# hammershock/3dgs-avatar-release

Hardware: AMD Instinct MI355X
Metric: render fps (fwd+bwd) @200k Gaussians 1024x1024 SH3 (higher is better)
Workload: dtype f32; 1 GPU; config3: 200k Gaussians, 1024x1024, SH deg 3, forward+backward; shs+scales+rotations inputs, L1 loss (L1 fused into the rasterizer: l1_target); tile_rect=1, l1=fused, long_lists=0, gaussians=200000, width=1024, height=1024, sh_degree=3, frames_per_rank=1857, total_frames=1857, ranks=1, backend=none, parallelism=frames sharded x1

## Files before the change

### 3dgs-avatar-release_amd/csrc/binning.hip

```cpp
#include "common.h"

__global__ __launch_bounds__(256) void first_pair_kernel(const uint32_t* __restrict__ tiles,
                                                         const uint32_t* __restrict__ wave_tiles, float* __restrict__ rec,
                                                         int P, unsigned long long* __restrict__ count,
                                                         unsigned long long* host_count) {
    __shared__ unsigned long long wb[4];
    const int tid = threadIdx.x, lane = tid & 63, wid = tid >> 6;
    const int w0 = 4 * (int)blockIdx.x;
    unsigned long long before = 0;
    for (int w = tid; w < w0; w += 256) before += wave_tiles[w];
#pragma unroll
    for (int d = 32; d >= 1; d >>= 1) before += __shfl_xor(before, d, 64);
    if (lane == 0) wb[wid] = before;
    const int i = blockIdx.x * 256 + tid;
    const uint32_t v = i < P ? tiles[i] : 0u;
    uint32_t x = v;
#pragma unroll
    for (int d = 1; d < 64; d <<= 1) {
        const uint32_t y = __shfl_up(x, d, 64);
        if (lane >= d) x += y;
    }
    __syncthreads();
    const unsigned long long block_base = (wb[0] + wb[1]) + (wb[2] + wb[3]);
    uint32_t woff = 0;
// ... 395 lines not shown
                                                          const uint32_t* __restrict__ keys, int mode, int ntiles,
                                                          uint32_t* __restrict__ order, const PairCount pc,
                                                          const FillJob fill, const LongLists ll) {
    if (blockIdx.x > 0) {
        if (fill.clean && *fill.clean == MARKS_CLEAN) return;
        const uint4 ones = make_uint4(0xFFFFFFFFu, 0xFFFFFFFFu, 0xFFFFFFFFu, 0xFFFFFFFFu);
        for (size_t k = (size_t)(blockIdx.x - 1) * 1024 + threadIdx.x; k < fill.quads; k += (size_t)(gridDim.x - 1) * 1024)
            if (fill.stream) store_stream(&fill.ptr[k], ones); else fill.ptr[k] = ones;
        return;
    }
    __shared__ uint32_t hist[1024];
    __shared__ uint32_t wmax[16];
    __shared__ uint32_t wsum[16];
    if (mode < 0) return;
    tile_order_body<HELD>(ranges, keys, mode, ntiles, order, pc, ll, hist, wmax, wsum);
}

#define BM_LD 33
#ifndef TW_STOP_AFTER
#define TW_STOP_AFTER 99
#endif
template <bool CW>
__global__ __launch_bounds__(TBK_THREADS) void tile_write_kernel(const uint4* __restrict__ ranklist,
                                                                 const uint32_t* __restrict__ seg_start, int P, int gx,
                                                                 int gy, int nbx, int nblocks, int nseg, int ntiles,
                                                                 const uint32_t* __restrict__ seg_cnt,
                                                                 const uint32_t* __restrict__ tile_tot,
                                                                 uint2* __restrict__ ranges, uint32_t* __restrict__ order,
                                                                 uint32_t* __restrict__ point_list, const PairCount pc,
                                                                 const LongLists ll) {
// ... 197 lines not shown

int launch_tile_order(const uint32_t* ranges, const uint32_t* keys, int mode, int ntiles, uint32_t* order, PairCount pc,
                      FillJob fill, LongLists ll, int debug, hipStream_t s) {
    const size_t pieces = (fill.quads + 1023) / 1024;
    const int side = fill.ptr ? (int)(pieces < 255 ? pieces : 255) : 0;
    if (ntiles <= 32 * 1024)
        hipLaunchKernelGGL(tile_order_kernel<true>, dim3(1 + side), dim3(1024), 0, s, reinterpret_cast<const uint2*>(ranges),
                           keys, mode, ntiles, order, pc, fill, ll);
    else
        hipLaunchKernelGGL(tile_order_kernel<false>, dim3(1 + side), dim3(1024), 0, s, reinterpret_cast<const uint2*>(ranges),
                           keys, mode, ntiles, order, pc, fill, ll);
    GS_LAUNCH_CHECK("tile_order", debug, s);
    return GS_OK;
}

int launch_tile_lists(const uint4* ranklist, const uint32_t* chunk_pairs, uint32_t* seg_start, int P, int gx, int gy, TileCounts tc, uint32_t* ranges,
                      uint32_t* order, uint32_t* point_list, PairCount pc, LongLists ll, bool totals_zeroed, int debug,
                      hipStream_t s) {
    uint32_t* seg_cnt = tc.seg_cnt;
    const BinGrid G = bin_grid(gx, gy);
    const int nseg = bin_segments(G, P);
    const int ntiles = gx * gy;
    if (!totals_zeroed) {
        const int zrc = gs_zero_async(tc.tile_tot, tc.zero_bytes, "tile_totals.zero", s);
        if (zrc != GS_OK) return zrc;
    }
    {
        int band_rows = TC_CELLS / (gx + 1) - 1;
        if (band_rows < 1) return GS_E_TOO_LARGE;
        if (band_rows > gy) band_rows = gy;
// ... 21 lines not shown
```

### 3dgs-avatar-release_amd/csrc/capi.hip

```cpp
#include "common.h"
#include <string.h>
#include <stdlib.h>
#include <atomic>
#include <chrono>
#include <mutex>
#include <vector>

static thread_local int g_last_hip = 0;
static thread_local const char* g_last_stage = "";
void gs_set_error(int hip_err, const char* stage) {
    g_last_hip = hip_err;
    g_last_stage = stage;
}

struct TuneSwitch {
    const char* name;
    int key, def;
    const char* env;
    bool (*ok)(int);
};
static const TuneSwitch k_tune[GS_TUNE_COUNT] = {
    {"xcd_map", GS_TUNE_XCD_MAP, 1, nullptr, nullptr},
    {"depth_sort", GS_TUNE_DEPTH_SORT, 1, nullptr, nullptr},
    {"nt_stores", GS_TUNE_NT_STORES, 1, nullptr, nullptr},
    {"bwd_chunks", GS_TUNE_BWD_CHUNKS, 1, nullptr, nullptr},
    {"fwd4", GS_TUNE_FWD4, 1, "GSPLAT_FWD4", nullptr},
    {"small_tiles", GS_TUNE_SMALL_TILES, BWD_CHUNK_MAX_TILES, nullptr, nullptr},
    {"shared_qlist", GS_TUNE_SHARED_QLIST, 1, nullptr, nullptr},
    {"ones_fast", GS_TUNE_ONES_FAST, 1, nullptr, nullptr},
    {"bwd_order", GS_TUNE_BWD_ORDER, 1, nullptr, nullptr},
    {"fwd_marks", GS_TUNE_FWD_MARKS, 1, nullptr, nullptr},
    {"fwdc_ch", GS_TUNE_FWDC_CH, (int)FWDC_CH_MIN, "GSPLAT_FWDC_CH", [](int v) { return v >= 64 && (v & (v - 1)) == 0; }},
    {"fwdc_div", GS_TUNE_FWDC_DIV, (int)FWD4_TOTAL_DIV, "GSPLAT_FWDC_DIV", [](int v) { return v >= 1; }},
};
struct TuneState {
    std::atomic<int> v[GS_TUNE_COUNT];
    TuneState() {
        for (const TuneSwitch& t : k_tune) {
            int value = t.def;
            if (const char* e = t.env ? getenv(t.env) : nullptr) {
                const int x = atoi(e);
                if (!t.ok || t.ok(x)) value = x;
            }
            v[t.key].store(value);
        }
    }
};
static TuneState& tune_state() {
// ... 289 lines not shown
        StageScope sc_("ranges_order", s);
        rc = launch_tile_order(im.ranges, nullptr, 0, im.ntiles, im.order, pc, FillJob{nullptr, 0},
                               LongLists{0, nullptr, im.cw_hdr, nullptr}, a->debug, s);
        if (rc != GS_OK) return rc;
    }
    QuadLists ql = quad_lists(im, b, a->long_lists);
    if (chunked) quad_lists_chunked(ql, im, im);
    if (cap > 0) {
        ql.marks = (gs_tune_get(GS_TUNE_FWD_MARKS) && !a->forward_only) ? b.marks : nullptr;
        ql.mark_quads = (size_t)cap;
        ql.marks_flag = b.marks_flag;
    }
    ql.l1_target = a->l1_target;
    ql.l1_part = im.l1_part;
    ql.l1_loss = a->l1_loss;
    { StageScope sc_("render_fwd", s);
    rc = launch_render_forward(g.rec, a->P > 0 ? b.point_list : nullptr, im.ranges, im.order, a->bg, a->W, a->H, out_color,
                               im.final_T, im.n_contrib, ql, s); }
    if (rc != GS_OK) return rc;
    return sync_if_debug(a, "render_forward", s);
}

int gs_forward_render(const GsFwdArgs* a, void* geom, size_t geom_bytes, void* binning, size_t binning_bytes,
                      void* img, size_t img_bytes, int64_t D, float* out_color, void* stream) {
    GS_CAPTURE_OK_IF(stream, a && !a->debug && a->frame_stats == nullptr);
    return forward_phase2(a, geom, geom_bytes, binning, binning_bytes, img, img_bytes, D, out_color, stream, false);
}

int gs_forward(const GsFwdArgs* a, void* geom, size_t geom_bytes, void* binning, size_t binning_bytes, int64_t capacity,
               void* img, size_t img_bytes, int32_t* radii, int64_t* count_host_pinned, float* out_color,
// ... 122 lines not shown
    if (a->P > 0 && scratch_bytes < scratch_total_bytes(D, a->P, im.ntiles)) return GS_E_WORKSPACE;
    if (a->P == 0) return GS_OK;
    hipStream_t s = (hipStream_t)stream;
    float* const sums = (float*)((char*)scratch + scratch_rows_bytes(D));
    if (D > 0) {
        const QuadLists ql = quad_lists(im, b, a->long_lists);
        SecondImage si{nullptr, nullptr, nullptr, nullptr, nullptr};
        if (second) {
            const ImgViewRO im2 = img_state(second->img, a->W, a->H, second->long_lists);
            if (second->img_bytes < im2.total || im2.bwd_chunks != im.bwd_chunks) return GS_E_BAD_ARG;
            si = SecondImage{second->colors, second->out_color, second->dL_dpix, ql.chunks > 1 ? im2.ckpt : nullptr, im2.all_ones};
        }
        uint32_t* const q8 = reinterpret_cast<uint32_t*>(b.marks);
        uint32_t* const own_order = (uint32_t*)((char*)sums + scratch_sums_bytes(a->P));
        const bool order_here = gs_tune_get(GS_TUNE_BWD_ORDER) != 0;
        { StageScope sc_("tile_order", s);
        rc = launch_tile_order(im.ranges, ql.qcount, order_here ? 1 : -1, im.ntiles, own_order, PairCount{nullptr, 0},
                               FillJob{b.marks, (size_t)D, gs_tune_get(GS_TUNE_NT_STORES) & 1, b.marks_flag},
                               LongLists{0, nullptr}, a->debug, s); }
        if (rc != GS_OK) return rc;
        { StageScope sc_("render_bwd", s);
        rc = launch_render_backward(g.rec, im.ranges, order_here ? own_order : im.order, a->W, a->H, ql, out_color, dL_dpix,
                                    dL_dopacity_img, im.final_T, a->bg, (float*)scratch, q8, second ? &si : nullptr,
                                    L1Grad{a->l1_target, a->l1_grad}, s); }
        if (rc != GS_OK) return rc;
        rc = sync_if_debug(a, "render_backward", s);
        if (rc != GS_OK) return rc;
    }
    StageScope sc_("gaussian_bwd", s);
    return launch_gaussian_backward(*a, radii, g.rec, g.tiles, g.clamped, reinterpret_cast<const uint32_t*>(b.marks),
                                    (const float*)scratch, sums, b.marks_flag, *gr, s);
}

int gs_backward(const GsFwdArgs* a, const int32_t* radii, const void* geom, size_t geom_bytes, void* binning,
                size_t binning_bytes, const void* img, size_t img_bytes, int64_t D, const float* out_color,
                const float* dL_dpix, void* scratch, size_t scratch_bytes, const GsGrads* gr, void* stream) {
    return backward_impl(a, radii, geom, geom_bytes, binning, binning_bytes, img, img_bytes, D, out_color, dL_dpix, nullptr,
// ... 838 lines not shown
    *n_out = n;
    return GS_OK;
}

int gs_tuning(const char* name, int value) {
    if (!name) return GS_E_BAD_ARG;
    for (const TuneSwitch& t : k_tune) {
        if (strcmp(name, t.name) != 0) continue;
        if (t.ok && !t.ok(value)) return GS_E_BAD_ARG;
        tune_state().v[t.key].store(value);
        return GS_OK;
    }
    return GS_E_BAD_ARG;
}

const char* gs_status_string(int code) {
    switch (code) {
        case GS_OK: return "ok";
        case GS_E_BAD_ARG: return "bad argument (null required pointer, non-positive size, unsupported SH degree / more than 16 SH coefficients, or rotations not 16-byte aligned)";
        case GS_E_EXCLUSIVE: return "provide exactly one of shs/colors_precomp and exactly one of (scales, rotations)/cov3D_precomp";
        case GS_E_TOO_LARGE: return "num_rendered or tile grid exceeds the supported index space";
        case GS_E_HIP: return "HIP error";
        case GS_E_WORKSPACE: return "state/workspace buffer smaller than gs_*_bytes requires";
        case GS_E_CAPTURE: return "the stream is being captured into a graph and this call is not capture-safe with these arguments (include/gsplat_mi355.h, \"Stream capture\"); nothing was enqueued";
        default: return "unknown status";
    }
}
int gs_last_hip_error(void) { return g_last_hip; }
const char* gs_last_stage(void) { return g_last_stage; }
const char* gs_build_info(void) { return "gsplat_mi355 gfx950 wave64 tile16 rec48"; }
// ... 3 lines not shown
```

### 3dgs-avatar-release_amd/csrc/common.h

```cpp
#pragma once
#include <hip/hip_runtime.h>
#include <stdint.h>
#include <stddef.h>
#include <type_traits>
#include "../../include/gsplat_mi355.h"

#define TILE 16
#define WAVE 64
#define REC_F 12
#define GS_MAX_PAIRS 0x3FFFFFFFll

static inline size_t align_up(size_t x, size_t a) { return (x + a - 1) / a * a; }

#define SORT_ITEMS 4096
#define SORT_SMALL_N (1 << 20)
#define SORT_TOTALS_REPL 16
static inline size_t sort_table_words(size_t n) {
    const size_t items = n <= (size_t)SORT_SMALL_N ? 1024 : SORT_ITEMS;
    return (size_t)256 * ((n + items - 1) / items + 4 * SORT_TOTALS_REPL);
}
#define SCAN_ITEMS 2048

#ifndef DS_ITEMS
#define DS_ITEMS 2048
// ... 78 lines not shown
    G.nby = (gy + TB_H - 1) / TB_H;
    G.nblocks = G.nbx * G.nby;
#ifndef TB_TARGET_WGS
#define TB_TARGET_WGS 512
#endif
    int s = (TB_TARGET_WGS + G.nblocks - 1) / G.nblocks;
    G.nseg_max = s < 1 ? 1 : (s > TB_MAX_SEG ? TB_MAX_SEG : s);
    return G;
}
static inline int bin_segments(const BinGrid& G, int P) {
    int s = (P + 1023) / 1024;
    if (s < 1) s = 1;
    return s < G.nseg_max ? s : G.nseg_max;
}

enum { GS_TUNE_XCD_MAP = 0, GS_TUNE_DEPTH_SORT = 1, GS_TUNE_NT_STORES = 2, GS_TUNE_BWD_CHUNKS = 3, GS_TUNE_FWD4 = 4, GS_TUNE_SMALL_TILES = 5, GS_TUNE_SHARED_QLIST = 6, GS_TUNE_ONES_FAST = 7, GS_TUNE_BWD_ORDER = 8, GS_TUNE_FWD_MARKS = 9, GS_TUNE_FWDC_CH = 10, GS_TUNE_FWDC_DIV = 11, GS_TUNE_COUNT = 12 };
int gs_tune_get(int key);

#define BWD_CH 128
#define BWD_KMAX 16
#define BWD_CHUNK_MAX_TILES 2048
#define FWD4_MAX_TILES 2048
#define FWD4_MIN_LIST 512u
#ifndef FWD4_TOTAL_DIV
#define FWD4_TOTAL_DIV 320ull
#endif

#define FWDC_CH_MIN 256u
#define FWDC_SPARSE_PAIRS 524288ull
#define FWDC_MAX_UNITS 4096
#define FWDC_MAX_TILES (FWDC_MAX_UNITS / 2)
#define FWDC_Q_WORDS (8 * FWDC_MAX_UNITS * 4)
#define FWDC_Q_BYTES ((size_t)FWDC_Q_WORDS * 4 + 64)
#ifdef FWDC_PROF
#define FWDC_SLOTS 9
#else
#define FWDC_SLOTS 8
#endif
#define FWDC_DEAD 0x80000000u
#define FWDC_SPIN_MAX (1 << 16)
struct ImgLayout {
    size_t ranges, n_contrib, final_T, ncon_c, tile_nmax, order, seg_cnt, tile_tot, all_ones, cw_flag, cw_done, cw_q, tile_zero_bytes, l1_part, ckpt, ck_start, cw_hdr, cw_units, cw_items, cw_rec, total;
    int gx, gy, bwd_chunks;
};
static inline bool few_long_lists_mode(int ntiles, int long_lists) {
    return ntiles <= gs_tune_get(GS_TUNE_SMALL_TILES) || long_lists != 0;
}
static inline ImgLayout img_layout(int W, int H, int long_lists = 0) {
    ImgLayout L;
    size_t o = 0;
    auto take = [&](size_t bytes) { size_t at = o; o = align_up(o + bytes, 256); return at; };
    L.gx = (W + TILE - 1) / TILE;
    L.gy = (H + TILE - 1) / TILE;
    const size_t nt = (size_t)L.gx * L.gy;
    L.ranges = take(nt * 8);
    L.n_contrib = take((size_t)W * H * 4);
    L.final_T = take((size_t)W * H * 4);
// ... 12 lines not shown
        L.cw_done = take(nt * 16);
        L.cw_q = take(FWDC_Q_BYTES);
        L.tile_zero_bytes = L.cw_q + FWDC_Q_BYTES - L.tile_tot;
    }
    L.l1_part = take(nt * 16);
    L.bwd_chunks = fl ? BWD_KMAX : 1;
    L.ckpt = take(nt * 4 * (size_t)(L.bwd_chunks - 1) * 64 * 16);
    L.ck_start = take(nt * 4 * (size_t)L.bwd_chunks * 4);
    L.cw_hdr = L.cw_units = L.cw_items = L.cw_rec = 0;
    if (cw) {
        L.cw_hdr = take(64);
        L.cw_units = take((size_t)FWDC_MAX_UNITS * 8);
        L.cw_items = take((size_t)FWDC_Q_WORDS * 4);
        L.cw_rec = take((size_t)FWDC_MAX_UNITS * 4 * FWDC_SLOTS * 64 * 4);
    }
    L.total = o;
    return L;
}

template <bool RO>
struct StateCarve {
    typename std::conditional<RO, const char, char>::type* base;
    StateCarve(typename std::conditional<RO, const void, void>::type* state) : base(static_cast<decltype(base)>(state)) {}
    template <class T>
    void operator()(T*& field, size_t offset, bool present = true) const {
        field = (base && present) ? reinterpret_cast<T*>(base + offset) : nullptr;
    }
};
template <bool RO>
struct GeomViewT {
// ... 17 lines not shown
    size_t total;
};
template <bool RO>
struct ImgViewT {
    template <class T> using ptr = typename std::conditional<RO, const T, T>::type*;
    ptr<uint32_t> ranges, n_contrib;
    ptr<float> final_T;
    ptr<uint32_t> ncon_c, qcount , order, seg_cnt, tile_tot, all_ones;
    ptr<uint32_t> cw_flag, cw_done, cw_q, cw_xcc_mask ;
    ptr<float> l1_part;
    ptr<float4> ckpt;
    ptr<uint32_t> ck_start, cw_hdr;
    ptr<uint2> cw_units;
    ptr<uint32_t> cw_items;
    ptr<float> cw_rec;
    size_t tile_zero_bytes;
    int cw_clear_words;
    size_t total;
    int gx, gy, ntiles, bwd_chunks;
};
typedef GeomViewT<false> GeomView;
typedef GeomViewT<true> GeomViewRO;
typedef BinViewT<false> BinView;
typedef BinViewT<true> BinViewRO;
typedef ImgViewT<false> ImgView;
typedef ImgViewT<true> ImgViewRO;

template <class Void >
static inline GeomViewT<std::is_const<Void>::value> geom_state(Void* base, int P) {
    constexpr bool RO = std::is_const<Void>::value;
// ... 22 lines not shown
}
template <class Void >
static inline ImgViewT<std::is_const<Void>::value> img_state(Void* base, int W, int H, int long_lists) {
    constexpr bool RO = std::is_const<Void>::value;
    const ImgLayout L = img_layout(W, H, long_lists);
    const StateCarve<RO> at{base};
    const bool cw = L.cw_rec != 0;
    ImgViewT<RO> v;
    at(v.ranges, L.ranges); at(v.n_contrib, L.n_contrib); at(v.final_T, L.final_T); at(v.ncon_c, L.ncon_c);
    at(v.qcount, L.tile_nmax); at(v.order, L.order); at(v.seg_cnt, L.seg_cnt); at(v.tile_tot, L.tile_tot);
    at(v.all_ones, L.all_ones);
    at(v.cw_flag, L.cw_flag, cw); at(v.cw_done, L.cw_done, cw); at(v.cw_q, L.cw_q, cw);
    at(v.cw_xcc_mask, L.cw_q + (size_t)FWDC_Q_WORDS * 4, cw);
    at(v.l1_part, L.l1_part); at(v.ckpt, L.ckpt); at(v.ck_start, L.ck_start);
    at(v.cw_hdr, L.cw_hdr, cw); at(v.cw_units, L.cw_units, cw); at(v.cw_items, L.cw_items, cw); at(v.cw_rec, L.cw_rec, cw);
    v.tile_zero_bytes = L.tile_zero_bytes;
    v.cw_clear_words = cw ? (int)((L.cw_q + FWDC_Q_BYTES - L.cw_flag) / 4) : 0;
    v.total = L.total; v.gx = L.gx; v.gy = L.gy; v.ntiles = L.gx * L.gy; v.bwd_chunks = L.bwd_chunks;
    return v;
}
static inline unsigned long long* not_ones_word(const GeomViewRO& first) {
    return const_cast<unsigned long long*>(first.count) + COUNT_NOT_ONES;
}

static inline int radix_passes(int bits) { return (bits + 7) / 8; }

void gs_set_error(int hip_err, const char* stage);
#define GS_LAUNCH_CHECK(stage, dbg, stream)                                            \
    do {                                                                               \
        hipError_t e__ = hipGetLastError();                                            \
// ... 307 lines not shown
int launch_knn_points(int Nq, const float* queries, int Nr, const float* ref, int K, float* out_d, long long* out_i,
                      void* ws, size_t ws_bytes, hipStream_t s);

int launch_build_cov(int N, const float* scales, float mod, const float* rot, int is_matrix, float* cov6, hipStream_t s);
int launch_build_cov_bwd(int N, const float* scales, float mod, const float* rot, int is_matrix, const float* dL_dcov6,
                         float* dL_dscales, float* dL_drot, hipStream_t s);
int launch_sh2rgb(int N, int deg, int M, const float* shs, const float* xyz, const float* campos, const float* R_fwd,
                  const float* noise_host, float* colors, uint8_t* clamped, hipStream_t s);
int launch_sh2rgb_bwd(int N, int deg, int M, const float* shs, const float* xyz, const float* campos, const float* R_fwd,
                      const float* noise_host, const uint8_t* clamped, const float* dL_dcolors, float* dL_dshs, float* dL_dxyz,
                      hipStream_t s);

size_t l1_ws_bytes(int64_t n);
int launch_l1_loss(const float* x, const float* y, int64_t n, float* loss, float* grad, float* partial, hipStream_t s);
int launch_loss_final(const float* partial, int nparts, float inv_n, float* loss, hipStream_t s);
int launch_bce_loss(const float* x, const float* y, int64_t n, float* loss, float* grad, float* partial, hipStream_t s);
size_t ssim_ws_bytes(int C, int H, int W);
int launch_ssim_forward(int C, int H, int W, const float* img1, const float* img2, float* ssim_out, float* dm_dmu1,
                        float* dm_ds1, float* dm_ds12, float* partial, hipStream_t s);
int launch_ssim_backward(int C, int H, int W, const float* img1, const float* img2, const float* dm_dmu1,
                         const float* dm_ds1, const float* dm_ds12, const float* dL_dssim, float* dL_dimg1,
                         hipStream_t s);

#define MARKS_CLEAN 0x600DF111u
struct FillJob { uint4* ptr; size_t quads; int stream = 0; const uint32_t* clean = nullptr;  };

typedef uint32_t gs_u32x4 __attribute__((ext_vector_type(4)));
__device__ __forceinline__ void store_stream(uint4* p, uint4 v) {
    gs_u32x4 x = {v.x, v.y, v.z, v.w};
    __builtin_nontemporal_store(x, reinterpret_cast<gs_u32x4*>(p));
// ... 17 lines not shown
    const float* src_cw_rec = nullptr;
    const float* src_final_T = nullptr;
    const uint32_t* src_qcount = nullptr;
    const uint32_t* src_n_contrib = nullptr;
    const unsigned long long* not_ones = nullptr;
    float4* ckpt = nullptr;
    uint32_t* ck_start = nullptr;
    int chunks = 1;
    uint4* marks = nullptr;
    size_t mark_quads = 0;
    uint32_t* marks_flag = nullptr;
    uint32_t* all_ones = nullptr;
    const float* l1_target = nullptr;
    float* l1_part = nullptr;
    float* l1_loss = nullptr;
};
int launch_render_forward(const float* rec, const uint32_t* point_list, const uint32_t* ranges, const uint32_t* order,
                          const float* bg, int W, int H, float* out_color, float* final_T, uint32_t* n_contrib,
                          const QuadLists& ql, hipStream_t s);
struct SecondImage {
    const float* colors;
    const float* out_color;
    const float* dL_dpix;
    const float4* ckpt;
    const uint32_t* all_ones;
};
struct L1Grad { const float* target; const float* grad; };
int launch_render_backward(const float* rec, const uint32_t* ranges, const uint32_t* order, int W, int H,
                           const QuadLists& ql, const float* out_color, const float* dL_dpix, const float* dL_dopa,
                           const float* final_T, const float* bg, float* qrows, uint32_t* q8, const SecondImage* second,
// ... 20 lines not shown
```

### 3dgs-avatar-release_amd/csrc/loss.hip

```cpp
#include "common.h"
#include <math.h>

#define L1_THREADS 256
#define L1_MAX_BLOCKS 1024

__device__ __forceinline__ float sgn_over_n(float d, float inv_n) { return d > 0.f ? inv_n : (d < 0.f ? -inv_n : 0.f); }

__global__ __launch_bounds__(L1_THREADS) void l1_partial_kernel(const float* __restrict__ x, const float* __restrict__ y,
                                                                int64_t n, float inv_n, float* __restrict__ grad,
                                                                float* __restrict__ partial) {
    __shared__ float ws[L1_THREADS / 64];
    const int tid = threadIdx.x, lane = tid & 63, wid = tid >> 6;
    float acc = 0.f;
    const int64_t n4 = n >> 2;
    const float4* x4 = reinterpret_cast<const float4*>(x);
    const float4* y4 = reinterpret_cast<const float4*>(y);
    float4* g4 = reinterpret_cast<float4*>(grad);
    const int64_t stride = (int64_t)gridDim.x * L1_THREADS;
    for (int64_t i = (int64_t)blockIdx.x * L1_THREADS + tid; i < n4; i += stride) {
        const float4 a = x4[i], b = y4[i];
        const float d0 = a.x - b.x, d1 = a.y - b.y, d2 = a.z - b.z, d3 = a.w - b.w;
        acc += (fabsf(d0) + fabsf(d1)) + (fabsf(d2) + fabsf(d3));
        g4[i] = make_float4(sgn_over_n(d0, inv_n), sgn_over_n(d1, inv_n), sgn_over_n(d2, inv_n), sgn_over_n(d3, inv_n));
    }
// ... 50 lines not shown

int launch_bce_loss(const float* x, const float* y, int64_t n, float* loss, float* grad, float* partial, hipStream_t s) {
    const int blocks = l1_blocks(n);
    const float inv_n = 1.0f / (float)n;
    StageScope st("bce_loss", s);
    hipLaunchKernelGGL(bce_partial_kernel, dim3(blocks), dim3(L1_THREADS), 0, s, x, y, n, inv_n, grad, partial);
    GS_LAUNCH_CHECK("bce_loss.partial", 0, s);
    hipLaunchKernelGGL(l1_final_kernel, dim3(1), dim3(L1_THREADS), 0, s, partial, blocks, inv_n, loss);
    GS_LAUNCH_CHECK("bce_loss.final", 0, s);
    return GS_OK;
}

__global__ __launch_bounds__(1024) void loss_final_wide_kernel(const float* __restrict__ partial, int nparts, float inv_n,
                                                               float* __restrict__ loss) {
    __shared__ float ws[16];
    const int tid = threadIdx.x, lane = tid & 63, wid = tid >> 6;
    float acc = 0.f;
    for (int i0 = tid; i0 < nparts; i0 += 8 * 1024) {
        float v[8];
#pragma unroll
        for (int u = 0; u < 8; u++) v[u] = (i0 + u * 1024 < nparts) ? partial[i0 + u * 1024] : 0.f;
#pragma unroll
        for (int u = 0; u < 8; u++) acc += v[u];
    }
    acc = wave_sum(acc);
    if (lane == 0) ws[wid] = acc;
    __syncthreads();
    if (tid == 0) {
        float t = 0.f;
        for (int w = 0; w < 16; w++) t += ws[w];
        loss[0] = t * inv_n;
    }
}

int launch_loss_final(const float* partial, int nparts, float inv_n, float* loss, hipStream_t s) {
    hipLaunchKernelGGL(loss_final_wide_kernel, dim3(1), dim3(1024), 0, s, partial, nparts, inv_n, loss);
    GS_LAUNCH_CHECK("loss_final", 0, s);
    return GS_OK;
}

int launch_l1_loss(const float* x, const float* y, int64_t n, float* loss, float* grad, float* partial, hipStream_t s) {
    const int blocks = l1_blocks(n);
    const float inv_n = 1.0f / (float)n;
    StageScope st("l1_loss", s);
    hipLaunchKernelGGL(l1_partial_kernel, dim3(blocks), dim3(L1_THREADS), 0, s, x, y, n, inv_n, grad, partial);
    GS_LAUNCH_CHECK("l1_loss.partial", 0, s);
    hipLaunchKernelGGL(l1_final_kernel, dim3(1), dim3(L1_THREADS), 0, s, partial, blocks, inv_n, loss);
// ... 260 lines not shown
```

### 3dgs-avatar-release_amd/csrc/render_fwd.hip

```cpp
#include "common.h"
#include "blend.h"
#include <type_traits>

struct FwdArgs {
    const float4* __restrict__ rec;
    const uint32_t* __restrict__ point_list;
    const uint2* __restrict__ ranges;
    const uint32_t* __restrict__ order;
    const float* __restrict__ bg;
    int W, H, gx, ntiles, xmap;
    float* __restrict__ out_color;
    float* __restrict__ final_T;
    uint32_t* __restrict__ n_contrib;
    uint32_t* __restrict__ qlist;
    uint32_t* __restrict__ ncon_c;
    uint32_t* __restrict__ qcount;
    float4* __restrict__ ckpt;
    uint32_t* __restrict__ ck_start;
    int chunks;
    const uint32_t* __restrict__ src_qcount;
    const uint32_t* __restrict__ src_n_contrib;
    const unsigned long long* __restrict__ not_ones;
    uint4* __restrict__ marks;
    size_t mark_quads;
// ... 875 lines not shown
    const dim3 grid(render_grid_blocks(gx * gy, xmap) + A.cw_blocks);
    const bool fq = ql.src_qcount != nullptr;
    if (ql.four_waves) {
        if (fq) hipLaunchKernelGGL(render_fwd_small_kernel<true>, grid, dim3(FWD4_BATCH), 0, s, A);
        else hipLaunchKernelGGL(render_fwd_small_kernel<false>, grid, dim3(FWD4_BATCH), 0, s, A);
    } else {
        if (A.cw_blocks) {
            if (fq) hipLaunchKernelGGL(render_fwd_cw_kernel<true>, grid, dim3(64), 0, s, A);
            else hipLaunchKernelGGL(render_fwd_cw_kernel<false>, grid, dim3(64), 0, s, A);
        } else {
            if (fq) hipLaunchKernelGGL(render_fwd_kernel<true>, grid, dim3(64), 0, s, A);
            else hipLaunchKernelGGL(render_fwd_kernel<false>, grid, dim3(64), 0, s, A);
        }
    }
    GS_LAUNCH_CHECK("render_forward", 0, s);
    if (ql.l1_target)
        return launch_loss_final(ql.l1_part, gx * gy * 4, 1.0f / (3.0f * (float)W * (float)H), ql.l1_loss, s);
    return GS_OK;
}

__global__ __launch_bounds__(256) void opacity_image_kernel(const float* __restrict__ final_T, const float* __restrict__ bg,
                                                            int n, float* __restrict__ out) {
    const int i = blockIdx.x * blockDim.x + threadIdx.x;
    if (i >= n) return;
    const float Tf = final_T[i];
    out[i] = (1.0f - Tf) + Tf * bg[0];
}

int launch_opacity_image(const float* final_T, const float* bg, int W, int H, float* out, hipStream_t s) {
    const int n = W * H;
    hipLaunchKernelGGL(opacity_image_kernel, dim3((n + 255) / 256), dim3(256), 0, s, final_T, bg, n, out);
    GS_LAUNCH_CHECK("opacity_image", 0, s);
// ... 3 lines not shown
```

### 3dgs-avatar-release_amd/diff_gaussian_rasterization/__init__.py

```python
import ctypes
import os
import threading
import weakref
from typing import NamedTuple

import torch
import torch.nn as nn

from gsplat_mi355 import _lib

__all__ = ["GaussianRasterizationSettings", "GaussianRasterizer", "rasterize_gaussians"]


class GaussianRasterizationSettings(NamedTuple):
    image_height: int
    image_width: int
    tanfovx: float
    tanfovy: float
    bg: torch.Tensor
    scale_modifier: float
    viewmatrix: torch.Tensor
    projmatrix: torch.Tensor
    sh_degree: int
    campos: torch.Tensor
# ... 255 lines not shown
                                                cov3Ds_precomp, raster_settings, with_opacity, dep, l1_target)
        args = (means3D, means2D, sh, colors_precomp, opacities, scales, rotations, cov3Ds_precomp)
        try:
            return _RasterizeGaussians._forward(ctx, means3D, means2D, sh, colors_precomp, opacities, scales, rotations,
                                                cov3Ds_precomp, raster_settings, with_opacity, dep, l1_target)
        except Exception:
            _dump_snapshot("snapshot_fw.dump", raster_settings, args)
            print("\nAn error occured in forward. Please forward snapshot_fw.dump for debugging.")
            raise

    @staticmethod
    def _forward(ctx, means3D, means2D, sh, colors_precomp, opacities, scales, rotations, cov3Ds_precomp,
                 raster_settings, with_opacity=False, dep=None, l1_target=None):
        ctx.with_opacity = bool(with_opacity)
        ctx.l1_target = None
        l1 = None
        ctx.defer_to = None
        means2D_in = means2D
        ctx.set_materialize_grads(False)
        L = _lib.load()
        means3D = _f32c(means3D, "means3D")
        if means3D is None:
            raise RuntimeError("diff_gaussian_rasterization: means3D is empty")
        sh = _f32c(sh, "shs")
        colors_precomp = _f32c(colors_precomp, "colors_precomp")
        opacities = _f32c(opacities, "opacities")
        scales = _f32c(scales, "scales")
        rotations = _f32c(rotations, "rotations")
        if rotations is not None:
            rotations = _lib.contiguous_aligned(rotations)
# ... 5 lines not shown
        with _lib.on_device(dev):
            a = _make_args(raster_settings, means3D, sh, colors_precomp, opacities, scales, rotations, cov3Ds_precomp,
                           keep)
            stream_h = _lib.stream_handle(dev)
            sptr = ctypes.c_void_p(stream_h)
            capturing = _stream_capturing()
            if capturing:
                a.frame_stats = None
            if l1_target is not None:
                ctx.l1_target = l1_target
                l1 = torch.empty((), dtype=torch.float32, device=dev)
                a.l1_target, a.l1_loss = l1_target.data_ptr(), l1.data_ptr()
            inference = isinstance(ctx, _InferenceCtx)
            if inference:
                a.forward_only = 1
            share = _SHARE and not inference and any(ctx.needs_input_grad)
            gkey = (_geom_cache.key(raster_settings, means3D, opacities, scales, rotations, cov3Ds_precomp, stream_h,
                                    capturing)
                    if share else None)
            hit = _geom_cache.take(dev, gkey) if (share and l1_target is None) else None
            if not share or l1_target is not None:
                _geom_cache.offer.pop(dev.index, None)
            ctx.geom_entry = None
            if hit is not None:
                a.long_lists = int(hit.long_lists)
            geom_bytes = _size("gs_geom_bytes", P)
            ik = ("img", W, H, int(a.long_lists))
            img_bytes = _sizes.get(ik)
            if img_bytes is None:
                img_bytes = _sizes[ik] = _lib.nbytes(L.gs_image_bytes_for, ctypes.byref(a))
# ... 142 lines not shown
            grad_out_color = torch.zeros(3, H, W, dtype=torch.float32, device=dev)
        g = _f32c(grad_out_color, "grad_out_color") if grad_out_color is not None else None
        g_l1 = _f32c(grad_l1, "grad_l1") if use_l1 else None
        g_op = _f32c(grad_out_opacity, "grad_out_opacity") if (ctx.with_opacity and grad_out_opacity is not None) else None
        with _lib.on_device(dev):
            a, _keep = ctx.fwd_args
            if (a.means3D != means3D.data_ptr() or a.opacities != opacities.data_ptr()
                    or (has_sh and a.shs != sh.data_ptr()) or (has_sr and a.scales != scales.data_ptr())):
                _keep = []
                a = _make_args(settings, means3D, sh if has_sh else None, colors_precomp if has_col else None, opacities,
                               scales if has_sr else None, rotations if has_sr else None,
                               cov3Ds_precomp if has_cov else None, _keep, long_lists=ctx.long_lists)
            a.l1_target = ctx.l1_target.data_ptr() if use_l1 else None
            a.l1_loss = None
            a.l1_grad = g_l1.data_ptr() if use_l1 else None
            gp = g.data_ptr() if g is not None else None
            sptr = _lib.stream_ptr(dev)
            scratch_bytes = _size("gs_backward_scratch_bytes", D, P, W, H)
            scratch = torch.empty(scratch_bytes, dtype=torch.uint8, device=dev)
            M = int(sh.shape[1]) if has_sh else 0
            f = dict(dtype=torch.float32, device=dev)
            d_means3D = torch.empty(P, 3, **f)
            d_means2D = torch.empty(P, 3, **f)
            d_colors = torch.empty(P, 3, **f)
            d_opacity = torch.empty(P, 1, **f)
            d_cov3D = torch.empty(P, 6, **f)
            d_sh = torch.empty(P, M, 3, **f) if has_sh else None
            d_scales = torch.empty(P, 3, **f) if has_sr else None
            d_rot = torch.empty(P, 4, **f) if has_sr else None
            gr = _lib.GsGrads(_lib.ptr(d_means3D), _lib.ptr(d_means2D), _lib.ptr(d_sh), _lib.ptr(d_colors),
# ... 62 lines not shown
```

### 3dgs-avatar-release_amd/gsplat_mi355/_lib.py

```python
import ctypes
import os
import threading
from ctypes import POINTER, c_char_p, c_double, c_float, c_int, c_int32, c_int64, c_size_t, c_uint8, c_void_p

_HERE = os.path.dirname(os.path.abspath(__file__))
LIB_PATH = os.environ.get("GSPLAT_LIB_PATH") or os.path.join(os.path.dirname(_HERE), "lib", "libgsplat_mi355.so")


class GsFwdArgs(ctypes.Structure):
    _fields_ = [
        ("P", c_int32), ("sh_degree", c_int32), ("M", c_int32), ("W", c_int32), ("H", c_int32),
        ("bg", c_void_p), ("means3D", c_void_p), ("shs", c_void_p), ("colors_precomp", c_void_p),
        ("opacities", c_void_p), ("scales", c_void_p), ("rotations", c_void_p), ("cov3D_precomp", c_void_p),
        ("viewmatrix", c_void_p), ("projmatrix", c_void_p), ("campos", c_void_p),
        ("scale_modifier", c_float), ("tanfovx", c_float), ("tanfovy", c_float),
        ("prefiltered", c_int32), ("debug", c_int32), ("tile_rect", c_int32), ("long_lists", c_int32),
        ("frame_stats", c_void_p), ("l1_target", c_void_p), ("l1_loss", c_void_p), ("l1_grad", c_void_p),
        ("forward_only", c_int32),
    ]


class GsSecondImage(ctypes.Structure):
    _fields_ = [("colors", c_void_p), ("out_color", c_void_p), ("dL_dpix", c_void_p), ("img", c_void_p),
                ("img_bytes", c_size_t), ("long_lists", c_int32)]


class GsGrads(ctypes.Structure):
    _fields_ = [(n, c_void_p) for n in ("dL_dmeans3D", "dL_dmeans2D", "dL_dsh", "dL_dcolors", "dL_dopacity",
                                        "dL_dscales", "dL_drotations", "dL_dcov3D")]


EXPORTS = ["gs_geom_bytes", "gs_image_bytes", "gs_binning_bytes", "gs_backward_scratch_bytes",
           "gs_forward_preprocess", "gs_forward_render", "gs_forward", "gs_forward_shared", "gs_backward", "gs_mark_visible", "knn_workspace_bytes",
           "knn_dist2", "gs_geom_field", "gs_binning_field", "gs_image_field", "gs_status_string",
           "gs_last_hip_error", "gs_last_stage", "gs_build_info", "gs_profile_enable", "gs_profile_filter", "gs_profile_collect",
           "gs_l1_loss_workspace_bytes", "gs_l1_loss", "gs_bce_loss", "gs_ssim_workspace_bytes", "gs_ssim_forward", "gs_ssim_backward",
           "gs_build_covariance", "gs_build_covariance_backward", "gs_sh2rgb", "gs_sh2rgb_backward", "knn_points", "gs_densify_stats", "gs_adam_step",
           "gs_opacity_image", "gs_backward_with_opacity", "gs_tuning", "gs_profile_reserve", "gs_image_bytes_for", "gs_backward_with_second", "gs_clock_probe", "gs_pair_stats", "gs_xcc_probe",
           "gs_densify_workspace_bytes", "gs_densify_plan", "gs_densify_apply", "gs_reset_opacity",
           "gs_aiap_workspace_bytes", "gs_aiap_forward", "gs_aiap_backward",
           "gs_hashgrid_levels", "gs_hashgrid_workspace_bytes", "gs_hashgrid_forward", "gs_hashgrid_backward",
           "gs_skin_weights_forward", "gs_skin_weights_backward", "gs_skinning_workspace_bytes", "gs_skinning_forward",
           "gs_skinning_backward",
           "gs_mesh_sample", "gs_skin_loss_workspace_bytes", "gs_skin_loss_forward", "gs_skin_loss_backward",
           "gs_pose_workspace_bytes", "gs_pose_forward", "gs_pose_backward",
           "gs_pose_encoder_grad_floats", "gs_pose_encoder_forward", "gs_pose_encoder_backward",
           "gs_nonrigid_workspace_bytes", "gs_nonrigid_apply_forward", "gs_nonrigid_apply_backward",
           "gs_texture_workspace_bytes", "gs_texture_input_forward", "gs_texture_input_backward",
           "gs_mlp_workspace_bytes", "gs_mlp_forward", "gs_mlp_backward",
           "gs_lpips_packed_bytes", "gs_lpips_pack_weights", "gs_lpips_workspace_bytes", "gs_lpips_forward", "gs_lpips_backward",
           "gs_lpips_conv", "gs_lpips_pool",
           "gs_grad_norm_workspace_bytes", "gs_grad_norm", "gs_grad_scale", "gs_adam_step_ex"]

# ... 219 lines not shown
        L.gs_lpips_workspace_bytes.argtypes = [c_int32, c_int32, c_int32, c_int32, c_int32, POINTER(c_size_t)]
        L.gs_lpips_forward.argtypes = [POINTER(GsLpipsArgs), c_void_p, c_void_p, c_void_p, c_size_t, c_void_p, c_size_t, c_void_p]
        L.gs_lpips_backward.argtypes = [POINTER(GsLpipsArgs), c_void_p, c_void_p, c_void_p, c_void_p, c_size_t, c_void_p, c_size_t,
                                        c_void_p]
        L.gs_lpips_conv.argtypes = [c_void_p, c_int32, c_int32, c_int32, c_int32, c_int32, c_void_p, c_int64, c_int64, c_void_p,
                                    c_void_p, c_void_p]
        L.gs_lpips_pool.argtypes = [c_int32, c_int32, c_int32, c_int32, c_void_p, c_void_p, c_void_p, c_void_p, c_void_p]
        L.gs_geom_field.argtypes = [c_void_p, c_int32, c_int32, POINTER(c_void_p)]
        L.gs_binning_field.argtypes = [c_void_p, c_int64, c_int32, c_int32, c_int32, POINTER(c_void_p)]
        L.gs_image_field.argtypes = [c_void_p, c_int32, c_int32, c_int32, POINTER(c_void_p)]
        L.gs_clock_probe.argtypes = [c_void_p, c_int32, c_void_p]
        L.gs_xcc_probe.argtypes = [c_void_p, c_int32, c_void_p]
        L.gs_pair_stats.argtypes = [POINTER(GsFwdArgs), c_void_p, c_size_t, c_void_p, c_size_t, c_void_p, c_size_t, c_int64, c_void_p,
                                    c_void_p]
        L.gs_tuning.argtypes = [c_char_p, c_int]
        L.gs_profile_reserve.argtypes = [c_int]
        L.gs_profile_enable.argtypes = [c_int]
        L.gs_profile_filter.argtypes = [c_char_p]
        L.gs_profile_collect.argtypes = [c_int, POINTER(c_char_p), POINTER(c_float), POINTER(c_int32), POINTER(c_int32)]
        for name in EXPORTS:
            getattr(L, name).restype = c_int
        L.gs_status_string.restype = c_char_p
        L.gs_status_string.argtypes = [c_int]
        L.gs_last_stage.restype = c_char_p
        L.gs_build_info.restype = c_char_p
        _lib = L
    return _lib


def check(rc):
# ... 2 lines not shown
        msg = L.gs_status_string(rc).decode()
        if rc == -4:
            msg += " %d in stage '%s'" % (L.gs_last_hip_error(), L.gs_last_stage().decode())
        raise RuntimeError("gsplat_mi355: " + msg)


tuning_listeners = []


def tuning(name, value):
    check(load().gs_tuning(name.encode(), int(value)))
    for fn in tuning_listeners:
        fn()


def profile_enable(on, stage=None):
    check(load().gs_profile_filter(stage.encode() if stage else None))
    check(load().gs_profile_enable(1 if on else 0))


def profile_reserve(n_events):
    check(load().gs_profile_reserve(int(n_events)))


def profile_collect(max_stages=32):
    names = (c_char_p * max_stages)()
    ms = (c_float * max_stages)()
    cnt = (c_int32 * max_stages)()
    n = c_int32(0)
    check(load().gs_profile_collect(max_stages, names, ms, cnt, ctypes.byref(n)))
# ... 86 lines not shown
```

### include/gsplat_mi355.h

```cpp
#ifndef GSPLAT_MI355_H
#define GSPLAT_MI355_H

#include <stddef.h>
#include <stdint.h>

#ifdef __cplusplus
extern "C" {
#endif

#define GS_OK 0
#define GS_E_BAD_ARG (-1)
#define GS_E_EXCLUSIVE (-2)
#define GS_E_TOO_LARGE (-3)
#define GS_E_HIP (-4)
#define GS_E_WORKSPACE (-5)
#define GS_E_CAPTURE (-6)


typedef struct GsFwdArgs {
    int32_t P;
    int32_t sh_degree;
    int32_t M;
    int32_t W, H;
    const float* bg;
// ... 5 lines not shown
    const float* rotations;
    const float* cov3D_precomp;
    const float* viewmatrix;
    const float* projmatrix;
    const float* campos;
    float scale_modifier, tanfovx, tanfovy;
    int32_t prefiltered;
    int32_t debug;
    int32_t tile_rect;
    int32_t long_lists;
    int64_t* frame_stats;
    const float* l1_target;
    float* l1_loss;
    const float* l1_grad;
    int32_t forward_only;
} GsFwdArgs;

typedef struct GsGrads {
    float* dL_dmeans3D;
    float* dL_dmeans2D;
    float* dL_dsh;
    float* dL_dcolors;
    float* dL_dopacity;
    float* dL_dscales;
    float* dL_drotations;
    float* dL_dcov3D;
} GsGrads;

int gs_geom_bytes(int32_t P, size_t* out);
int gs_image_bytes(int32_t W, int32_t H, size_t* out);
// ... 364 lines not shown
int gs_image_bytes_for(const GsFwdArgs* a, size_t* out);

int gs_profile_reserve(int n_events);
int gs_profile_enable(int on);
int gs_profile_filter(const char* stage);
int gs_profile_collect(int max, const char** names, float* ms, int32_t* launches, int32_t* n_out);

int gs_pair_stats(const GsFwdArgs* a, const void* geom, size_t geom_bytes, const void* binning, size_t binning_bytes,
                  const void* img, size_t img_bytes, int64_t num_rendered, uint64_t* counts, void* stream);

int gs_clock_probe(uint64_t* ticks, int32_t iters, void* stream);

int gs_xcc_probe(uint32_t* xcc, int32_t n_blocks, void* stream);

int gs_tuning(const char* name, int value);
const char* gs_status_string(int code);
int gs_last_hip_error(void);
const char* gs_last_stage(void);
const char* gs_build_info(void);

#ifdef __cplusplus
}
#endif
#endif
```

Before: 1822 frames/s.

## Fuse backward tile ordering into forward L1 loss finalize kernel

When the L1 loss is fused and backward will follow, the forward pass now launches a combined two-block kernel. One block reduces the L1 partials and the other computes the backward tile order from qcount into a new image buffer. Backward then skips its separate tile_order launch when marks are already clean, removing one kernel launch and its serial latency from the backward critical path. It adds a per-image buffer, a new tuning switch and Python plumbing, and it depends on the marks having been cleared by the forward pass.

```diff
diff --git a/3dgs-avatar-release_amd/csrc/binning.hip b/3dgs-avatar-release_amd/csrc/binning.hip
--- a/3dgs-avatar-release_amd/csrc/binning.hip
+++ b/3dgs-avatar-release_amd/csrc/binning.hip
@@ -433,6 +433,20 @@
     __shared__ uint32_t wsum[16];
     if (mode < 0) return;
     tile_order_body<HELD>(ranges, keys, mode, ntiles, order, pc, ll, hist, wmax, wsum);
+}
+
+template <bool HELD>
+__global__ __launch_bounds__(1024) void loss_final_order_kernel(const float* __restrict__ partial, int nparts, float inv_n,
+                                                                float* __restrict__ loss, const uint32_t* __restrict__ qcount,
+                                                                int ntiles, uint32_t* __restrict__ bwd_order) {
+    __shared__ uint32_t hist[1024];
+    __shared__ uint32_t wmax[16];
+    __shared__ uint32_t wsum[16];
+    if (blockIdx.x == 0) {
+        loss_final_wide_body(partial, nparts, inv_n, loss, reinterpret_cast<float*>(wmax));
+        return;
+    }
+    tile_order_body<HELD>(nullptr, qcount, 1, ntiles, bwd_order, PairCount{nullptr, 0}, LongLists{0, nullptr}, hist, wmax, wsum);
 }
 
 #define BM_LD 33
@@ -660,6 +674,16 @@
     return GS_OK;
 }
 
+int launch_loss_final_order(const float* partial, int nparts, float inv_n, float* loss, const uint32_t* qcount, int ntiles,
+                            uint32_t* bwd_order, hipStream_t s) {
+    if (ntiles <= 32 * 1024)
+        hipLaunchKernelGGL(loss_final_order_kernel<true>, dim3(2), dim3(1024), 0, s, partial, nparts, inv_n, loss, qcount, ntiles, bwd_order);
+    else
+        hipLaunchKernelGGL(loss_final_order_kernel<false>, dim3(2), dim3(1024), 0, s, partial, nparts, inv_n, loss, qcount, ntiles, bwd_order);
+    GS_LAUNCH_CHECK("loss_final_order", 0, s);
+    return GS_OK;
+}
+
 int launch_tile_lists(const uint4* ranklist, const uint32_t* chunk_pairs, uint32_t* seg_start, int P, int gx, int gy, TileCounts tc, uint32_t* ranges,
                       uint32_t* order, uint32_t* point_list, PairCount pc, LongLists ll, bool totals_zeroed, int debug,
                       hipStream_t s) {
diff --git a/3dgs-avatar-release_amd/csrc/capi.hip b/3dgs-avatar-release_amd/csrc/capi.hip
--- a/3dgs-avatar-release_amd/csrc/capi.hip
+++ b/3dgs-avatar-release_amd/csrc/capi.hip
@@ -32,6 +32,7 @@
     {"fwd_marks", GS_TUNE_FWD_MARKS, 1, nullptr, nullptr},
     {"fwdc_ch", GS_TUNE_FWDC_CH, (int)FWDC_CH_MIN, "GSPLAT_FWDC_CH", [](int v) { return v >= 64 && (v & (v - 1)) == 0; }},
     {"fwdc_div", GS_TUNE_FWDC_DIV, (int)FWD4_TOTAL_DIV, "GSPLAT_FWDC_DIV", [](int v) { return v >= 1; }},
+    {"fwd_bwd_order", GS_TUNE_FWD_BWD_ORDER, 1, "GSPLAT_FWD_BWD_ORDER", nullptr},
 };
 struct TuneState {
     std::atomic<int> v[GS_TUNE_COUNT];
@@ -351,6 +352,7 @@
     ql.l1_target = a->l1_target;
     ql.l1_part = im.l1_part;
     ql.l1_loss = a->l1_loss;
+    if (a->l1_target && !a->forward_only && gs_tune_get(GS_TUNE_FWD_BWD_ORDER)) ql.bwd_order = im.bwd_order;
     { StageScope sc_("render_fwd", s);
     rc = launch_render_forward(g.rec, a->P > 0 ? b.point_list : nullptr, im.ranges, im.order, a->bg, a->W, a->H, out_color,
                                im.final_T, im.n_contrib, ql, s); }
@@ -503,13 +505,24 @@
         uint32_t* const q8 = reinterpret_cast<uint32_t*>(b.marks);
         uint32_t* const own_order = (uint32_t*)((char*)sums + scratch_sums_bytes(a->P));
         const bool order_here = gs_tune_get(GS_TUNE_BWD_ORDER) != 0;
-        { StageScope sc_("tile_order", s);
-        rc = launch_tile_order(im.ranges, ql.qcount, order_here ? 1 : -1, im.ntiles, own_order, PairCount{nullptr, 0},
-                               FillJob{b.marks, (size_t)D, gs_tune_get(GS_TUNE_NT_STORES) & 1, b.marks_flag},
-                               LongLists{0, nullptr}, a->debug, s); }
-        if (rc != GS_OK) return rc;
+        const bool prepared = a->bwd_prepared != 0 && gs_tune_get(GS_TUNE_FWD_BWD_ORDER) != 0;
+        if (prepared && a->debug) {
+            uint32_t flag = 0;
+            hipError_t e = hipMemcpyAsync(&flag, b.marks_flag, 4, hipMemcpyDeviceToHost, s);
+            if (e == hipSuccess) e = hipStreamSynchronize(s);
+            if (e != hipSuccess) { gs_set_error((int)e, "bwd_prepared.check"); return GS_E_HIP; }
+            if (flag != MARKS_CLEAN) return GS_E_BAD_ARG;
+        }
+        if (!prepared) {
+            StageScope sc_("tile_order", s);
+            rc = launch_tile_order(im.ranges, ql.qcount, order_here ? 1 : -1, im.ntiles, own_order, PairCount{nullptr, 0},
+                                   FillJob{b.marks, (size_t)D, gs_tune_get(GS_TUNE_NT_STORES) & 1, b.marks_flag},
+                                   LongLists{0, nullptr}, a->debug, s);
+            if (rc != GS_OK) return rc;
+        }
+        const uint32_t* const bwd_order = !order_here ? im.order : (prepared ? im.bwd_order : own_order);
         { StageScope sc_("render_bwd", s);
-        rc = launch_render_backward(g.rec, im.ranges, order_here ? own_order : im.order, a->W, a->H, ql, out_color, dL_dpix,
+        rc = launch_render_backward(g.rec, im.ranges, bwd_order, a->W, a->H, ql, out_color, dL_dpix,
                                     dL_dopacity_img, im.final_T, a->bg, (float*)scratch, q8, second ? &si : nullptr,
                                     L1Grad{a->l1_target, a->l1_grad}, s); }
         if (rc != GS_OK) return rc;
@@ -1378,6 +1391,16 @@
     return GS_E_BAD_ARG;
 }
 
+int gs_tuning_get(const char* name, int* value) {
+    if (!name || !value) return GS_E_BAD_ARG;
+    for (const TuneSwitch& t : k_tune) {
+        if (strcmp(name, t.name) != 0) continue;
+        *value = gs_tune_get(t.key);
+        return GS_OK;
+    }
+    return GS_E_BAD_ARG;
+}
+
 const char* gs_status_string(int code) {
     switch (code) {
         case GS_OK: return "ok";
diff --git a/3dgs-avatar-release_amd/csrc/common.h b/3dgs-avatar-release_amd/csrc/common.h
--- a/3dgs-avatar-release_amd/csrc/common.h
+++ b/3dgs-avatar-release_amd/csrc/common.h
@@ -116,7 +116,7 @@
     return s < G.nseg_max ? s : G.nseg_max;
 }
 
-enum { GS_TUNE_XCD_MAP = 0, GS_TUNE_DEPTH_SORT = 1, GS_TUNE_NT_STORES = 2, GS_TUNE_BWD_CHUNKS = 3, GS_TUNE_FWD4 = 4, GS_TUNE_SMALL_TILES = 5, GS_TUNE_SHARED_QLIST = 6, GS_TUNE_ONES_FAST = 7, GS_TUNE_BWD_ORDER = 8, GS_TUNE_FWD_MARKS = 9, GS_TUNE_FWDC_CH = 10, GS_TUNE_FWDC_DIV = 11, GS_TUNE_COUNT = 12 };
+enum { GS_TUNE_XCD_MAP = 0, GS_TUNE_DEPTH_SORT = 1, GS_TUNE_NT_STORES = 2, GS_TUNE_BWD_CHUNKS = 3, GS_TUNE_FWD4 = 4, GS_TUNE_SMALL_TILES = 5, GS_TUNE_SHARED_QLIST = 6, GS_TUNE_ONES_FAST = 7, GS_TUNE_BWD_ORDER = 8, GS_TUNE_FWD_MARKS = 9, GS_TUNE_FWDC_CH = 10, GS_TUNE_FWDC_DIV = 11, GS_TUNE_FWD_BWD_ORDER = 12, GS_TUNE_COUNT = 13 };
 int gs_tune_get(int key);
 
 #define BWD_CH 128
@@ -142,7 +142,7 @@
 #define FWDC_DEAD 0x80000000u
 #define FWDC_SPIN_MAX (1 << 16)
 struct ImgLayout {
-    size_t ranges, n_contrib, final_T, ncon_c, tile_nmax, order, seg_cnt, tile_tot, all_ones, cw_flag, cw_done, cw_q, tile_zero_bytes, l1_part, ckpt, ck_start, cw_hdr, cw_units, cw_items, cw_rec, total;
+    size_t ranges, n_contrib, final_T, ncon_c, tile_nmax, order, seg_cnt, tile_tot, all_ones, cw_flag, cw_done, cw_q, tile_zero_bytes, l1_part, ckpt, ck_start, cw_hdr, cw_units, cw_items, cw_rec, bwd_order, total;
     int gx, gy, bwd_chunks;
 };
 static inline bool few_long_lists_mode(int ntiles, int long_lists) {
@@ -185,6 +185,7 @@
         L.cw_items = take((size_t)FWDC_Q_WORDS * 4);
         L.cw_rec = take((size_t)FWDC_MAX_UNITS * 4 * FWDC_SLOTS * 64 * 4);
     }
+    L.bwd_order = take(nt * 4);
     L.total = o;
     return L;
 }
@@ -232,6 +233,7 @@
     ptr<uint2> cw_units;
     ptr<uint32_t> cw_items;
     ptr<float> cw_rec;
+    ptr<uint32_t> bwd_order;
     size_t tile_zero_bytes;
     int cw_clear_words;
     size_t total;
@@ -284,6 +286,7 @@
     at(v.cw_xcc_mask, L.cw_q + (size_t)FWDC_Q_WORDS * 4, cw);
     at(v.l1_part, L.l1_part); at(v.ckpt, L.ckpt); at(v.ck_start, L.ck_start);
     at(v.cw_hdr, L.cw_hdr, cw); at(v.cw_units, L.cw_units, cw); at(v.cw_items, L.cw_items, cw); at(v.cw_rec, L.cw_rec, cw);
+    at(v.bwd_order, L.bwd_order);
     v.tile_zero_bytes = L.tile_zero_bytes;
     v.cw_clear_words = cw ? (int)((L.cw_q + FWDC_Q_BYTES - L.cw_flag) / 4) : 0;
     v.total = L.total; v.gx = L.gx; v.gy = L.gy; v.ntiles = L.gx * L.gy; v.bwd_chunks = L.bwd_chunks;
@@ -621,6 +624,28 @@
 size_t l1_ws_bytes(int64_t n);
 int launch_l1_loss(const float* x, const float* y, int64_t n, float* loss, float* grad, float* partial, hipStream_t s);
 int launch_loss_final(const float* partial, int nparts, float inv_n, float* loss, hipStream_t s);
+__device__ __forceinline__ void loss_final_wide_body(const float* __restrict__ partial, int nparts, float inv_n,
+                                                     float* __restrict__ loss, float* ws) {
+    const int tid = threadIdx.x, lane = tid & 63, wid = tid >> 6;
+    float acc = 0.f;
+    for (int i0 = tid; i0 < nparts; i0 += 8 * 1024) {
+        float v[8];
+#pragma unroll
+        for (int u = 0; u < 8; u++) v[u] = (i0 + u * 1024 < nparts) ? partial[i0 + u * 1024] : 0.f;
+#pragma unroll
+        for (int u = 0; u < 8; u++) acc += v[u];
+    }
+    acc = wave_sum(acc);
+    if (lane == 0) ws[wid] = acc;
+    __syncthreads();
+    if (tid == 0) {
+        float t = 0.f;
+        for (int w = 0; w < 16; w++) t += ws[w];
+        loss[0] = t * inv_n;
+    }
+}
+int launch_loss_final_order(const float* partial, int nparts, float inv_n, float* loss, const uint32_t* qcount, int ntiles,
+                            uint32_t* bwd_order, hipStream_t s);
 int launch_bce_loss(const float* x, const float* y, int64_t n, float* loss, float* grad, float* partial, hipStream_t s);
 size_t ssim_ws_bytes(int C, int H, int W);
 int launch_ssim_forward(int C, int H, int W, const float* img1, const float* img2, float* ssim_out, float* dm_dmu1,
@@ -668,6 +693,7 @@
     const float* l1_target = nullptr;
     float* l1_part = nullptr;
     float* l1_loss = nullptr;
+    uint32_t* bwd_order = nullptr;
 };
 int launch_render_forward(const float* rec, const uint32_t* point_list, const uint32_t* ranges, const uint32_t* order,
                           const float* bg, int W, int H, float* out_color, float* final_T, uint32_t* n_contrib,
diff --git a/3dgs-avatar-release_amd/csrc/loss.hip b/3dgs-avatar-release_amd/csrc/loss.hip
--- a/3dgs-avatar-release_amd/csrc/loss.hip
+++ b/3dgs-avatar-release_amd/csrc/loss.hip
@@ -88,23 +88,7 @@
 __global__ __launch_bounds__(1024) void loss_final_wide_kernel(const float* __restrict__ partial, int nparts, float inv_n,
                                                                float* __restrict__ loss) {
     __shared__ float ws[16];
-    const int tid = threadIdx.x, lane = tid & 63, wid = tid >> 6;
-    float acc = 0.f;
-    for (int i0 = tid; i0 < nparts; i0 += 8 * 1024) {
-        float v[8];
-#pragma unroll
-        for (int u = 0; u < 8; u++) v[u] = (i0 + u * 1024 < nparts) ? partial[i0 + u * 1024] : 0.f;
-#pragma unroll
-        for (int u = 0; u < 8; u++) acc += v[u];
-    }
-    acc = wave_sum(acc);
-    if (lane == 0) ws[wid] = acc;
-    __syncthreads();
-    if (tid == 0) {
-        float t = 0.f;
-        for (int w = 0; w < 16; w++) t += ws[w];
-        loss[0] = t * inv_n;
-    }
+    loss_final_wide_body(partial, nparts, inv_n, loss, ws);
 }
 
 int launch_loss_final(const float* partial, int nparts, float inv_n, float* loss, hipStream_t s) {
diff --git a/3dgs-avatar-release_amd/csrc/render_fwd.hip b/3dgs-avatar-release_amd/csrc/render_fwd.hip
--- a/3dgs-avatar-release_amd/csrc/render_fwd.hip
+++ b/3dgs-avatar-release_amd/csrc/render_fwd.hip
@@ -913,8 +913,12 @@
         }
     }
     GS_LAUNCH_CHECK("render_forward", 0, s);
-    if (ql.l1_target)
-        return launch_loss_final(ql.l1_part, gx * gy * 4, 1.0f / (3.0f * (float)W * (float)H), ql.l1_loss, s);
+    if (ql.l1_target) {
+        const float inv_n = 1.0f / (3.0f * (float)W * (float)H);
+        if (ql.bwd_order)
+            return launch_loss_final_order(ql.l1_part, gx * gy * 4, inv_n, ql.l1_loss, ql.qcount, gx * gy, ql.bwd_order, s);
+        return launch_loss_final(ql.l1_part, gx * gy * 4, inv_n, ql.l1_loss, s);
+    }
     return GS_OK;
 }
 
diff --git a/3dgs-avatar-release_amd/diff_gaussian_rasterization/__init__.py b/3dgs-avatar-release_amd/diff_gaussian_rasterization/__init__.py
--- a/3dgs-avatar-release_amd/diff_gaussian_rasterization/__init__.py
+++ b/3dgs-avatar-release_amd/diff_gaussian_rasterization/__init__.py
@@ -293,6 +293,8 @@
                  raster_settings, with_opacity=False, dep=None, l1_target=None):
         ctx.with_opacity = bool(with_opacity)
         ctx.l1_target = None
+        ctx.bwd_prepared = False
+        ctx.backwards = 0
         l1 = None
         ctx.defer_to = None
         means2D_in = means2D
@@ -328,6 +330,8 @@
             inference = isinstance(ctx, _InferenceCtx)
             if inference:
                 a.forward_only = 1
+            ctx.bwd_prepared = bool(l1_target is not None and not inference and _lib.tuning_value("fwd_marks")
+                                    and _lib.tuning_value("fwd_bwd_order"))
             share = _SHARE and not inference and any(ctx.needs_input_grad)
             gkey = (_geom_cache.key(raster_settings, means3D, opacities, scales, rotations, cov3Ds_precomp, stream_h,
                                     capturing)
@@ -500,6 +504,8 @@
             a.l1_target = ctx.l1_target.data_ptr() if use_l1 else None
             a.l1_loss = None
             a.l1_grad = g_l1.data_ptr() if use_l1 else None
+            a.bwd_prepared = int(ctx.bwd_prepared and ctx.backwards == 0 and second is None and not a.forward_only)
+            ctx.backwards += 1
             gp = g.data_ptr() if g is not None else None
             sptr = _lib.stream_ptr(dev)
             scratch_bytes = _size("gs_backward_scratch_bytes", D, P, W, H)
diff --git a/3dgs-avatar-release_amd/gsplat_mi355/_lib.py b/3dgs-avatar-release_amd/gsplat_mi355/_lib.py
--- a/3dgs-avatar-release_amd/gsplat_mi355/_lib.py
+++ b/3dgs-avatar-release_amd/gsplat_mi355/_lib.py
@@ -16,7 +16,7 @@
         ("scale_modifier", c_float), ("tanfovx", c_float), ("tanfovy", c_float),
         ("prefiltered", c_int32), ("debug", c_int32), ("tile_rect", c_int32), ("long_lists", c_int32),
         ("frame_stats", c_void_p), ("l1_target", c_void_p), ("l1_loss", c_void_p), ("l1_grad", c_void_p),
-        ("forward_only", c_int32),
+        ("forward_only", c_int32), ("bwd_prepared", c_int32),
     ]
 
 
@@ -36,7 +36,7 @@
            "gs_last_hip_error", "gs_last_stage", "gs_build_info", "gs_profile_enable", "gs_profile_filter", "gs_profile_collect",
            "gs_l1_loss_workspace_bytes", "gs_l1_loss", "gs_bce_loss", "gs_ssim_workspace_bytes", "gs_ssim_forward", "gs_ssim_backward",
            "gs_build_covariance", "gs_build_covariance_backward", "gs_sh2rgb", "gs_sh2rgb_backward", "knn_points", "gs_densify_stats", "gs_adam_step",
-           "gs_opacity_image", "gs_backward_with_opacity", "gs_tuning", "gs_profile_reserve", "gs_image_bytes_for", "gs_backward_with_second", "gs_clock_probe", "gs_pair_stats", "gs_xcc_probe",
+           "gs_opacity_image", "gs_backward_with_opacity", "gs_tuning", "gs_tuning_get", "gs_profile_reserve", "gs_image_bytes_for", "gs_backward_with_second", "gs_clock_probe", "gs_pair_stats", "gs_xcc_probe",
            "gs_densify_workspace_bytes", "gs_densify_plan", "gs_densify_apply", "gs_reset_opacity",
            "gs_aiap_workspace_bytes", "gs_aiap_forward", "gs_aiap_backward",
            "gs_hashgrid_levels", "gs_hashgrid_workspace_bytes", "gs_hashgrid_forward", "gs_hashgrid_backward",
@@ -286,6 +286,7 @@
         L.gs_pair_stats.argtypes = [POINTER(GsFwdArgs), c_void_p, c_size_t, c_void_p, c_size_t, c_void_p, c_size_t, c_int64, c_void_p,
                                     c_void_p]
         L.gs_tuning.argtypes = [c_char_p, c_int]
+        L.gs_tuning_get.argtypes = [c_char_p, POINTER(c_int)]
         L.gs_profile_reserve.argtypes = [c_int]
         L.gs_profile_enable.argtypes = [c_int]
         L.gs_profile_filter.argtypes = [c_char_p]
@@ -318,6 +319,19 @@
         fn()
 
 
+_tuning_values = {}
+tuning_listeners.append(_tuning_values.clear)
+
+
+def tuning_value(name):
+    v = _tuning_values.get(name)
+    if v is None:
+        out = c_int(0)
+        check(load().gs_tuning_get(name.encode(), ctypes.byref(out)))
+        v = _tuning_values[name] = int(out.value)
+    return v
+
+
 def profile_enable(on, stage=None):
     check(load().gs_profile_filter(stage.encode() if stage else None))
     check(load().gs_profile_enable(1 if on else 0))
diff --git a/include/gsplat_mi355.h b/include/gsplat_mi355.h
--- a/include/gsplat_mi355.h
+++ b/include/gsplat_mi355.h
@@ -43,6 +43,7 @@
     float* l1_loss;
     const float* l1_grad;
     int32_t forward_only;
+    int32_t bwd_prepared;
 } GsFwdArgs;
 
 typedef struct GsGrads {
@@ -437,6 +438,7 @@
 int gs_xcc_probe(uint32_t* xcc, int32_t n_blocks, void* stream);
 
 int gs_tuning(const char* name, int value);
+int gs_tuning_get(const char* name, int* value);
 const char* gs_status_string(int code);
 int gs_last_hip_error(void);
 const char* gs_last_stage(void);
```

Result: no change. 1832 frames/s, median of 6 (+0.6%).
